# ChainBreak/denoising_diffusion_deep_fake

Hardware: NVIDIA B200
Metric: train_img_per_s (higher is better)
Workload: dtype bf16

## Files before the change

denoising_diffusion_deep_fake_b200/csrc/api.cu:

```cuda
#include <stdarg.h>
#include <string.h>
#include <stdlib.h>
#include "common.cuh"

namespace d3fk {

int64_t g_launch_count = 0;
char g_last_error[512] = "";
int* g_dev_error_flag = nullptr;
int g_use_pdl = 1;
static int g_inited_device = -1;

int set_error(int code, const char* fmt, ...) {
  va_list ap;
  va_start(ap, fmt);
  vsnprintf(g_last_error, sizeof(g_last_error), fmt, ap);
  va_end(ap);
  return code;
}

int check_launch(const char* what) {
  cudaError_t e = cudaPeekAtLastError();
  if (e != cudaSuccess) {
    cudaGetLastError();
// ... 27 lines not shown
int launch_chansum(const d3fk_chansum_params*, cudaStream_t);
int launch_upcat(const d3fk_upcat_params*, cudaStream_t);
int launch_frames_to_tensor(const d3fk_frames_params*, cudaStream_t);
int launch_tensor_to_frames(const d3fk_frames_params*, cudaStream_t);
int launch_affine_qsample(const d3fk_affine_qsample_params*, cudaStream_t);
int launch_qsample(const d3fk_qsample_params*, cudaStream_t);
int launch_posterior(const d3fk_posterior_params*, cudaStream_t);
int launch_inc(const d3fk_misc_params*, cudaStream_t);
int launch_adam(const d3fk_adam_params*, cudaStream_t);
int launch_set_scalars(const d3fk_scalars_params*, cudaStream_t);
int launch_pack_all(const d3fk_misc_params*, cudaStream_t);
int launch_loss(const d3fk_loss_params*, cudaStream_t);
int loss_init();
int tc_init();

static int require_init() {
  if (g_inited_device < 0) return set_error(D3FK_ERR_ARCH, "d3fk_init() has not succeeded on an sm_100 device");
  return D3FK_OK;
}

static int conv_dispatch(const d3fk_conv_params* p, cudaStream_t s) {
  if (p->dtype == D3FK_F32) {
    if (p->mode == 2) return set_error(D3FK_ERR_UNSUPPORTED, "conv mode 2 (windowed rows) is a bf16-engine path");
    return launch_conv_ffma(p, s);
  }
  if (p->dtype == D3FK_BF16) return launch_conv_tc(p, s);
  return set_error(D3FK_ERR_ARG, "conv: bad dtype %d", p->dtype);
}
static int wgrad_dispatch(const d3fk_wgrad_params* p, cudaStream_t s) {
  if (p->dtype == D3FK_F32) {
    if (p->mode == 2) return set_error(D3FK_ERR_UNSUPPORTED, "wgrad mode 2 (space-to-depth stem) is a bf16-engine path");
    return launch_wgrad_ffma(p, s);
  }
  if (p->dtype == D3FK_BF16) return launch_wgrad_tc(p, s);
  return set_error(D3FK_ERR_ARG, "wgrad: bad dtype %d", p->dtype);
}

static int wgrad_group_dispatch(const d3fk_wgrad_group_params* p, cudaStream_t s) {
  if (p->base.dtype == D3FK_BF16) return launch_wgrad_group_tc(p, s);
  if (p->count < 1 || p->count > D3FK_WGRAD_GROUP_MAX) return set_error(D3FK_ERR_ARG, "wgrad group: count %d", p->count);
  for (int i = 0; i < p->count; ++i) {
    d3fk_wgrad_params one = p->base;
    one.src0 = p->src0[i]; one.dy = p->dy[i]; one.dw = p->dw[i];
    int rc = wgrad_dispatch(&one, s);
    if (rc) return rc;
  }
// ... 297 lines not shown
```

denoising_diffusion_deep_fake_b200/csrc/conv_tc.cu:

```cuda
#include "tc_common.cuh"

namespace d3fk {

template <int BN, int PATH, int FUSE> struct ConvCfg {
  static constexpr int STAGES = BN >= 128 ? ((PATH == 2 && FUSE == 3) ? 6 : 3) : 4;
  static constexpr int B_STAGE_BYTES = BN * 128;
  static constexpr int SMEM = 1024 + STAGES * (A_STAGE_BYTES + B_STAGE_BYTES) + 256 + 10 * BN * 4;
  static constexpr int ACC_COLS = BN < 32 ? 32 : BN;
  static constexpr int TMEM_COLS = 2 * ACC_COLS;
};

struct TileSched {
  int MT, NT, KS, kb_per_split, nkb, total, a_ca;
  int bw, bh, bn, wt, ht;
  int off_w, off_h;
  int a_pitch;
};

__device__ __forceinline__ void decode_tile(const TileSched& ts, int t, int& mt, int& nt, int& ks) {
  if (ts.KS > 1) {
    ks = t % ts.KS;
    const int r = t / ts.KS;
    mt = r % ts.MT;
    nt = r / ts.MT;
  } else {
    ks = 0;
    mt = t % ts.MT;
    nt = t / ts.MT;
  }
}

struct FuseBN {
  const float* gamma; const float* beta;
  float* mean; float* invstd; float* running_mean; float* running_var; long long* nbt;
  float* scale; float* shift;
  bf16* act; const bf16* res;
  unsigned* barrier;
  long long count;
  int ldact, ldr, relu;
  float eps, momentum;
};

template <int BN, int PATH, int FUSE>
__global__ void __launch_bounds__(TC_THREADS, 2) conv_tc_kernel(Gather g, FastDiv dWo, FastDiv dHo, const __grid_constant__ CUtensorMap tmA,
                                                             const __grid_constant__ CUtensorMap tmB, EpiTC e, TileSched ts,
                                                             FuseBN fb, int* errflag) {
  using Cfg = ConvCfg<BN, PATH, FUSE>;
  constexpr int STAGES = Cfg::STAGES;
  constexpr int CW = BN >= 32 ? 32 : 16;
  extern __shared__ uint8_t smem_raw[];
  const uint32_t base = (smem_u32(smem_raw) + 1023u) & ~1023u;
  const uint32_t a_base = base;
  const uint32_t b_base = base + STAGES * A_STAGE_BYTES;
  const uint32_t bar_base = b_base + STAGES * Cfg::B_STAGE_BYTES;
  uint8_t* gen_bar = smem_raw + (base - smem_u32(smem_raw)) + STAGES * (A_STAGE_BYTES + Cfg::B_STAGE_BYTES);
  volatile uint32_t* tmem_ptr_slot = reinterpret_cast<volatile uint32_t*>(gen_bar + 8 * (2 * STAGES + 4));
  float* s_stat = reinterpret_cast<float*>(gen_bar + 256);
  float* s_aff = s_stat + 8 * BN;
  constexpr bool affine = FUSE == 3;
  auto full_bar = [&](int s) { return bar_base + 8u * s; };
  auto empty_bar = [&](int s) { return bar_base + 8u * (STAGES + s); };
  auto acc_full_bar = [&](int b) { return bar_base + 8u * (2 * STAGES + b); };
  auto acc_empty_bar = [&](int b) { return bar_base + 8u * (2 * STAGES + 2 + b); };
  const uint32_t recv_bar = bar_base + 8u * (2 * STAGES + 5);

  const int tid = threadIdx.x, warp = warp_index_uniform(), lane = tid & 31;
// ... 21 lines not shown
      mbar_init(empty_bar(s), 1);
    }
    for (int b = 0; b < 2; ++b) {
      mbar_init(acc_full_bar(b), 1);
      mbar_init(acc_empty_bar(b), EPI_THREADS);
    }
    mbar_init(recv_bar, 1);
    fence_barrier_init();
  }
  if (is_epi) {
    for (int i = etid; i < 8 * BN; i += EPI_THREADS) s_stat[i] = 0.f;
  }
  if (warp == 5 && elect_one_sync()) {
    tma_prefetch_desc(&tmB);
    if (PATH == 2) tma_prefetch_desc(&tmA);
    int mt0, nt0, ks0;
    decode_tile(ts, blockIdx.x, mt0, nt0, ks0);
    const int kbp = ks0 * ts.kb_per_split;
    for (int i = 0; i < STAGES && kbp + i < ts.nkb; ++i) tma_prefetch_l2_2d(&tmB, (kbp + i) * TC_BK, nt0 * BN);
  }
  if (FUSE == 2 && is_epi && e.bw_x) {
    int mt0, nt0, ks0;
    decode_tile(ts, blockIdx.x, mt0, nt0, ks0);
    const long long mp = (long long)mt0 * TC_BM + q * 32 + lane;
    if (mp < g.M) {
      for (int b = half * 128; b < BN * 2; b += 256) {
        prefetch_l2(reinterpret_cast<const char*>(e.bw_x + mp * e.bw_ldx + nt0 * BN) + b);
        if (e.bw_relu) prefetch_l2(reinterpret_cast<const char*>(e.bw_act + mp * e.bw_ldact + nt0 * BN) + b);
      }
    }
  }
  if (warp == 4) tmem_alloc(smem_u32((const void*)tmem_ptr_slot), Cfg::TMEM_COLS);
  tc_fence_before();
  __syncthreads();
  tc_fence_after();
  const uint32_t tmem_d = *tmem_ptr_slot;
  if (tid == 0) { TL_STAMP(1) }

  auto flush_stats = [&](int nt) {
    asm volatile("bar.sync 1, 256;" ::: "memory");
    const int n0 = nt * BN;
    if (tid < BN && n0 + tid < e.Cout) {
      const float a = (s_stat[tid] + s_stat[2 * BN + tid]) + (s_stat[4 * BN + tid] + s_stat[6 * BN + tid]);
      const float b = (s_stat[BN + tid] + s_stat[3 * BN + tid]) + (s_stat[5 * BN + tid] + s_stat[7 * BN + tid]);
      if (a != 0.f || b != 0.f) {
        atomicAdd(&e.stats[n0 + tid], (double)a);
        atomicAdd(&e.stats[e.Cout + n0 + tid], (FUSE == 2 && e.bw_x) ? bw_second_sum((double)a, (double)b, e, n0 + tid) : (double)b);
      }
// ... 46 lines not shown
        for (int i = 0; i < 8; ++i) y[i] += __bfloat162float(rb16[i]);
      }
      if (fb.relu) {
#pragma unroll
        for (int i = 0; i < 8; ++i) y[i] = fmaxf(y[i], 0.f);
      }
      uint4 o;
      __nv_bfloat162* o2 = reinterpret_cast<__nv_bfloat162*>(&o);
#pragma unroll
      for (int i = 0; i < 4; ++i) o2[i] = __floats2bfloat162_rn(y[2 * i], y[2 * i + 1]);
      *reinterpret_cast<uint4*>(fb.act + m * fb.ldact + cbase + q * 8) = o;
    }
  };

  if (warp == 5) {
    pdl_enter();
    if (tid == 160) { TL_STAMP(2) }
    if (elect_one_sync()) {
      uint32_t kbg = 0;
      const int sgn = g.mode ? -1 : 1;
      for (int t = blockIdx.x; t < ts.total; t += gridDim.x) {
        int mt, nt, ks;
        decode_tile(ts, t, mt, nt, ks);
        const int kb0 = ks * ts.kb_per_split;
        const int kb1 = min(ts.nkb, kb0 + ts.kb_per_split);
        int w0 = 0, h0 = 0, i0 = 0, tap = 0, c = 0, khi = 0, kwi = 0;
        if (PATH == 2) {
          const int tw = mt % ts.wt;
          const int r2 = mt / ts.wt;
          w0 = tw * ts.bw + ts.off_w;
          h0 = (r2 % ts.ht) * ts.bh + ts.off_h;
          i0 = (r2 / ts.ht) * ts.bn;
          const int k = kb0 * TC_BK;
          tap = k / g.ctot;
          c = k - tap * g.ctot;
          khi = tap / g.kw;
          kwi = tap - khi * g.kw;
        }
        for (int kb = kb0; kb < kb1; ++kb, ++kbg) {
          const int s = kbg % STAGES;
          if (kbg >= STAGES) mbar_wait(empty_bar(s), ((kbg / STAGES) - 1) & 1, errflag);
          mbar_arrive_expect_tx(full_bar(s), Cfg::B_STAGE_BYTES + (PATH == 2 ? A_STAGE_BYTES : 0));
          tma_load_2d(b_base + s * Cfg::B_STAGE_BYTES, &tmB, kb * TC_BK, nt * BN, full_bar(s));
          if (PATH == 2) {
            tma_load_4d(a_base + s * A_STAGE_BYTES, &tmA, c, w0 + sgn * kwi, h0 + sgn * khi, i0, full_bar(s));
            c += TC_BK;
            if (c >= g.ctot) {
              c = 0;
              if (++kwi == g.kw) { kwi = 0; ++khi; }
            }
          }
        }
      }
    }
    __syncwarp();
    if (clus) cluster_sync_relaxed();
  } else if (warp == 4) {
    pdl_enter();
    if (elect_one_sync()) {
      constexpr uint32_t idesc = make_idesc(TC_BM, BN, 0, 0);
      uint32_t kbg = 0, tile_iter = 0;
      for (int t = blockIdx.x; t < ts.total; t += gridDim.x, ++tile_iter) {
        int mt, nt, ks;
        decode_tile(ts, t, mt, nt, ks);
        const int kb0 = ks * ts.kb_per_split;
        const int kb1 = min(ts.nkb, kb0 + ts.kb_per_split);
        const uint32_t abuf = tile_iter & 1;
        if (tile_iter >= 2) {
          mbar_wait(acc_empty_bar(abuf), ((tile_iter >> 1) - 1) & 1, errflag);
          tc_fence_after();
        }
        const uint32_t d_addr = tmem_d + abuf * Cfg::ACC_COLS;
        for (int kb = kb0; kb < kb1; ++kb, ++kbg) {
          const int s = kbg % STAGES;
          mbar_wait(full_bar(s), (kbg / STAGES) & 1, errflag);
          if (kbg == 0) { TL_STAMP(3) }
          tc_fence_after();
          const uint32_t a_addr = a_base + s * A_STAGE_BYTES;
          const uint32_t b_addr = b_base + s * Cfg::B_STAGE_BYTES;
#pragma unroll
          for (int kk = 0; kk < TC_BK / 16; ++kk) {
            uint64_t ad = make_smem_desc(a_addr + kk * 32, 16, 1024);
            uint64_t bd = make_smem_desc(b_addr + kk * 32, 16, 1024);
            umma_f16(d_addr, ad, bd, idesc, (kb > kb0 || kk > 0) ? 1u : 0u);
          }
          umma_commit(empty_bar(s));
        }
        umma_commit(acc_full_bar(abuf));
        TL_STAMP(4)
      }
    }
    __syncwarp();
    if (clus) cluster_sync_relaxed();
  } else {
    const int j = tid & 7;
    const int rb = tid >> 3;
    const uint32_t sw = (uint32_t)((j ^ (rb & 7)) << 4);
    const int sgn = g.mode ? -1 : 1;
    const uint32_t smask = g.mode ? (uint32_t)(g.stride - 1) : 0u;
    const int sshift = g.mode ? g.sshift : 0;
    const int row = q * 32 + lane;
#pragma unroll 1
    for (int pass = 0; pass < 2; ++pass) {
      int pass_v = pass;
      asm volatile("" : "+r"(pass_v));
      const bool live = pass_v != 0;
      if (live) {
        pdl_enter();
        if (tid == 0) { TL_STAMP(2) }
      }
      uint32_t kbg = 0;
      uint32_t tile_iter = 0;
      int cur_nt = -1, cur_aff_nt = -1;
      for (int t = blockIdx.x; t < ts.total; t += gridDim.x, ++tile_iter) {
        int mt, nt, ks;
        decode_tile(ts, t, mt, nt, ks);
        const int m0 = mt * TC_BM, n0 = nt * BN;
        const int kb0 = ks * ts.kb_per_split;
        const int kb1 = min(ts.nkb, kb0 + ts.kb_per_split);

        if (PATH != 2 && warp < 4 && live) {
          int rh[8], rw[8];
          int rn[8];
          const bf16* rp[8];
#pragma unroll
          for (int i = 0; i < 8; ++i) {
            const int m = m0 + rb + 16 * i;
            int n = 0, h0 = -(1 << 28), w0 = 0;
            if (m < g.M) {
              const uint32_t qq = fdiv((uint32_t)m, dWo);
              const int wo = m - (int)qq * g.Wo;
              n = (int)fdiv(qq, dHo);
              const int ho = (int)qq - n * g.Ho;
              if (g.mode == 0) { h0 = ho * g.stride - g.pad; w0 = wo * g.stride - g.pad; }
              else { h0 = ho + g.pad; w0 = wo + g.pad; }
            }
            rh[i] = h0; rw[i] = w0;
            if (PATH == 0) rp[i] = (const bf16*)g.src0 + ((long long)(n * g.Hi + h0) * g.Wi + w0) * g.ld0;
            else rn[i] = n;
          }
          int k = kb0 * TC_BK + j * 8;
          int tap = k / g.ctot;
// ... 31 lines not shown
                if (ts.a_ca) cp_async_16_ca(a_dst + i * (16 * 128), src, ok ? 16u : 0u);
                else cp_async_16(a_dst + i * (16 * 128), src, ok ? 16u : 0u);
              }
            }
            cp_async_mbar_arrive(full_bar(s));
            mbar_arrive(full_bar(s));
            k += TC_BK;
            c += TC_BK;
            while (c >= g.ctot) {
              c -= g.ctot;
              if (++kwi == g.kw) { kwi = 0; ++khi; }
            }
          }
        }

        const uint32_t abuf = tile_iter & 1;
        if (live) {
          mbar_wait(acc_full_bar(abuf), (tile_iter >> 1) & 1, errflag);
          if (tid == 0) { TL_STAMP(5) }
          tc_fence_after();
        }
        const int m = m0 + row;
        const bool row_ok = live && m < g.M;
        if (!clus) {
          if (affine && (cur_aff_nt != nt || !live)) {
            stage_affine(nt, live);
            cur_aff_nt = live ? nt : -1;
          }
          if (live && do_stats && cur_nt != nt) {
            if (cur_nt >= 0) flush_stats(cur_nt);
            cur_nt = nt;
          }
          int on = 0, oh = 0, ow = 0;
          if (e.out_nchw && row_ok) {
            const uint32_t qq = fdiv((uint32_t)m, dWo);
            ow = m - (int)qq * e.Wo;
            on = (int)fdiv(qq, dHo);
            oh = (int)qq - on * e.Ho;
          }
#pragma unroll 1
          for (int cc = half * CW; cc < BN; cc += 2 * CW) {
            uint32_t raw[CW];
            const uint32_t taddr = tmem_d + ((uint32_t)(q * 32) << 16) + abuf * Cfg::ACC_COLS + (uint32_t)cc;
            const bool tstats = do_stats && !(FUSE == 2 && e.bw_x);
            if (tstats) tmem_col_stats<CW>(taddr, live ? g.M - (m0 + q * 32) : 0, s_stat + q * 2 * BN + cc, s_stat + q * 2 * BN + BN + cc, lane);
            if (CW == 32) tmem_ld32(taddr, raw); else tmem_ld16(taddr, raw);
            tmem_ld_wait();
            float f[CW];
#pragma unroll
            for (int i = 0; i < CW; ++i) f[i] = __uint_as_float(raw[i]);
            epilogue_chunk<CW, FUSE == 2>(f, e, (long long)m, row_ok, n0 + cc, on, oh, ow, do_stats && !tstats, s_stat + q * 2 * BN + cc,
                                          s_stat + q * 2 * BN + BN + cc, lane, affine ? s_aff + cc : nullptr, BN);
            if (tid == 0 && cc == 0) { TL_STAMP(8) }
          }
          if (tid == 0) { TL_STAMP(9) }
          if (FUSE == 1 && live) {
            flush_stats(nt);
            cur_nt = -1;
            fuse_finalize(nt, mt == 0);
#pragma unroll 1
            for (int cc = half * CW; cc < BN; cc += 2 * CW) {
              uint32_t raw[CW];
              const uint32_t taddr = tmem_d + ((uint32_t)(q * 32) << 16) + abuf * Cfg::ACC_COLS + (uint32_t)cc;
              if (CW == 32) tmem_ld32(taddr, raw); else tmem_ld16(taddr, raw);
              tmem_ld_wait();
              float f[CW];
#pragma unroll
              for (int i = 0; i < CW; ++i) f[i] = __uint_as_float(raw[i]);
              fuse_apply(f, CW, (long long)m, row_ok, nt, cc);
            }
          }
          if (live) {
            tc_fence_before();
            mbar_arrive(acc_empty_bar(abuf));
          }
        } else {
          const int KS = ts.KS, SL = BN / KS, sl4 = SL >> 2;
          const uint32_t rank = cluster_ctarank();
          const uint32_t recv = a_base;
          if (live) {
            if (etid == 0) mbar_arrive_expect_tx(recv_bar, (uint32_t)(TC_BM * BN * 4));
            tc_fence_before();
            cluster_sync_relaxed();
            tc_fence_after();
            if (tid == 0) { TL_STAMP(11) }
          }
#pragma unroll 1
          for (int cc = half * CW; cc < BN; cc += 2 * CW) {
            uint32_t raw[CW];
            const uint32_t taddr = tmem_d + ((uint32_t)(q * 32) << 16) + (uint32_t)cc;
            if (CW == 32) tmem_ld32(taddr, raw); else tmem_ld16(taddr, raw);
            tmem_ld_wait();
#pragma unroll
            for (int q4 = 0; q4 < CW / 4; ++q4) {
              const int col = cc + 4 * q4;
              const int owner = col / SL, within = col - owner * SL;
              const uint32_t la = recv + (uint32_t)((((int)rank * sl4 + (within >> 2)) * 128 + row) * 16);
              const uint32_t ra = mapa_shared(la, (uint32_t)owner);
              if (live) st_async_f4(ra, raw[4 * q4], raw[4 * q4 + 1], raw[4 * q4 + 2], raw[4 * q4 + 3], mapa_shared(recv_bar, (uint32_t)owner));
            }
          }
          if (live) {
            if (tid == 0) { TL_STAMP(12) }
            mbar_wait(recv_bar, 0, errflag);
            if (tid == 0) { TL_STAMP(13) }
          }
          if (affine) stage_affine(nt, live);
          const int cslice = (int)rank * SL;
#pragma unroll 1
          for (int ch = half * 16; ch < SL; ch += 32) {
            float f[16];
#pragma unroll
            for (int c4 = 0; c4 < 4; ++c4) {
              float4 a = make_float4(0.f, 0.f, 0.f, 0.f);
              for (int r = 0; r < KS; ++r) {
                const float4 v = ld_shared_f4(recv + (uint32_t)(((r * sl4 + (ch >> 2) + c4) * 128 + row) * 16));
                a.x += v.x; a.y += v.y; a.z += v.z; a.w += v.w;
              }
              f[4 * c4] = a.x; f[4 * c4 + 1] = a.y; f[4 * c4 + 2] = a.z; f[4 * c4 + 3] = a.w;
            }
            const int ct = cslice + ch;
            const bool tstats = do_stats && !(FUSE == 2 && e.bw_x);
            if (tstats) {
              const uint32_t taddr = tmem_d + ((uint32_t)(q * 32) << 16) + (uint32_t)ct;
              if (live) tmem_st16(taddr, f);
              __syncwarp();
              tmem_col_stats<16>(taddr, live ? g.M - (m0 + q * 32) : 0, s_stat + q * 2 * BN + ct, s_stat + q * 2 * BN + BN + ct, lane);
            }
            epilogue_chunk<16, FUSE == 2>(f, e, (long long)m, row_ok, nt * BN + ct, 0, 0, 0, do_stats && !tstats, s_stat + q * 2 * BN + ct,
                                          s_stat + q * 2 * BN + BN + ct, lane, affine ? s_aff + ct : nullptr, BN);
          }
          if (tid == 0) { TL_STAMP(14) }
          if (live && do_stats) flush_stats(nt);
          if (tid == 0) { TL_STAMP(15) }
          if (FUSE == 1 && live) {
            fuse_finalize(nt, mt == 0 && rank == 0);
#pragma unroll 1
            for (int ch = half * 16; ch < SL; ch += 32) {
              float f[16];
#pragma unroll
              for (int c4 = 0; c4 < 4; ++c4) {
                float4 a = make_float4(0.f, 0.f, 0.f, 0.f);
                for (int r = 0; r < KS; ++r) {
                  const float4 v = ld_shared_f4(recv + (uint32_t)(((r * sl4 + (ch >> 2) + c4) * 128 + row) * 16));
                  a.x += v.x; a.y += v.y; a.z += v.z; a.w += v.w;
                }
                f[4 * c4] = a.x; f[4 * c4 + 1] = a.y; f[4 * c4 + 2] = a.z; f[4 * c4 + 3] = a.w;
              }
              fuse_apply(f, 16, (long long)m, row_ok, nt, cslice + ch);
            }
          }
        }
// ... 5 lines not shown
  }

  if (tid == 0) { TL_STAMP(6) }
  tc_fence_before();
  __syncthreads();
  if (warp == 4) tmem_dealloc(tmem_d, Cfg::TMEM_COLS);
  if (tid == 128) { TL_STAMP(7) }
}

int g_num_sms = 148;
int g_verbose = 0;
int g_max_cluster = 8;
static int g_tile_loop = 1;
static int g_a_ca = 0;
static int g_occ_cap = 0;
static int g_use_tma_a = 1;
static int g_split_tiles = 74;
static int g_split_cta_cap = 100;

struct FuseReq { const d3fk_bn_params* bn; unsigned* barrier; bool taken; };
static thread_local FuseReq* t_fuse = nullptr;
static int g_fuse_bn = 1;

template <int BN, int PATH>
static int launch_conv_tc_bn(const Gather& g, const d3fk_conv_params* p, cudaStream_t s, const TileSched& box) {
  EpiTC e{(bf16*)p->out, p->out_nchw, p->scale, p->shift, (const bf16*)p->res, p->stats, p->ldo, p->ldr, p->relu, p->Cout, p->Ho, p->Wo,
           (const bf16*)p->bw_x, (const bf16*)p->bw_act, p->bw_mean, p->bw_invstd, p->bw_ldx, p->bw_ldact, p->bw_relu};
  TileSched ts = box;
  ts.MT = cdiv(g.M, TC_BM);
  ts.NT = cdiv(p->Cout, BN);
  ts.nkb = cdiv(g.K, TC_BK);
  ts.KS = 1;
  const int tiles = ts.MT * ts.NT;
  ts.a_ca = g_a_ca && p->kh > 1;
  if (BN == 128 && !p->out_nchw && p->Cout % BN == 0 && tiles <= g_split_tiles && ts.nkb >= 8 && g_max_cluster > 1) {
    int ks = 1;
    while (ks * 2 <= g_max_cluster && ks * 2 <= 8 && tiles * ks * 2 <= g_split_cta_cap * g_num_sms / 100 && ts.nkb / (ks * 2) >= 4) ks *= 2;
    while (ks > 1 && tiles * ks > cluster_capacity(ks, 2)) ks >>= 1;
    ts.KS = ks;
  }
  ts.kb_per_split = cdiv(ts.nkb, ts.KS);
  if (ts.KS > 1 && (ts.KS - 1) * ts.kb_per_split >= ts.nkb) {
    ts.KS = 1;
    ts.kb_per_split = ts.nkb;
  }
  ts.total = tiles * ts.KS;
  const bool eval_affine = !p->bw_x && (p->scale || p->shift);
  const int smem_bytes = eval_affine ? ConvCfg<BN, PATH, 3>::SMEM : ConvCfg<BN, PATH, 0>::SMEM;
  int occ = (227 * 1024) / (smem_bytes + 1024);
  if (occ * ConvCfg<BN, PATH, 0>::TMEM_COLS > 512) occ = 512 / ConvCfg<BN, PATH, 0>::TMEM_COLS;
  if (g_occ_cap > 0 && occ > g_occ_cap) occ = g_occ_cap;
  int grid = ts.total < g_num_sms * occ ? ts.total : g_num_sms * occ;
  if (!g_tile_loop || ts.KS > 1) grid = ts.total;

  alignas(64) CUtensorMap tmA, tmB;
  memset(&tmA, 0, sizeof(tmA));
  {
    uint64_t dims[2] = {(uint64_t)g.K, (uint64_t)p->Cout};
    uint64_t strides[1] = {(uint64_t)g.K * 2};
    uint32_t bx[2] = {TC_BK, (uint32_t)BN};
// ... 3 lines not shown
  if (PATH == 2) {
    uint64_t dims[4] = {(uint64_t)g.c0, (uint64_t)g.Wi, (uint64_t)g.Hi, (uint64_t)g.B};
    const uint64_t pitch = (uint64_t)(ts.a_pitch ? ts.a_pitch : g.Wi);
    uint64_t strides[3] = {(uint64_t)g.ld0 * 2, pitch * g.ld0 * 2, (uint64_t)g.Hi * pitch * g.ld0 * 2};
    uint32_t bx[4] = {TC_BK, (uint32_t)ts.bw, (uint32_t)ts.bh, (uint32_t)ts.bn};
    int rc = get_tensor_map(&tmA, p->src0, 4, dims, strides, bx, 128);
    if (rc) return rc;
  }
  FuseBN fb;
  memset(&fb, 0, sizeof(fb));
  bool fuse = false;
  if (BN == 128 && t_fuse && g_fuse_bn && p->stats && !p->scale && !p->shift && !p->res && !p->relu && !p->out_nchw && p->mode == 0 &&
      p->Cout % BN == 0 && ts.total <= cluster_capacity_safe(ts.KS)) {
    const d3fk_bn_params* b = t_fuse->bn;
    fb.gamma = b->gamma; fb.beta = b->beta; fb.mean = b->mean; fb.invstd = b->invstd; fb.scale = b->scale; fb.shift = b->shift;
    fb.running_mean = b->running_mean; fb.running_var = b->running_var; fb.nbt = (long long*)b->num_batches_tracked;
    fb.act = (bf16*)b->y; fb.res = (const bf16*)b->res; fb.barrier = t_fuse->barrier; fb.count = b->count;
    fb.ldact = b->ldy; fb.ldr = b->ldr; fb.relu = b->relu; fb.eps = b->eps; fb.momentum = b->momentum;
    fuse = true;
    grid = ts.total;
    t_fuse->taken = true;
  }
  const int epi = p->bw_x ? 2 : fuse ? 1 : (p->scale || p->shift) ? 3 : 0;
  if (g_verbose) fprintf(stderr, "[d3fk] conv<%d,%d> mode=%d M=%d K=%d Cout=%d tiles=%d KS=%d kbps=%d grid=%d fuse=%d epi=%d\n", BN, PATH, g.mode, g.M, g.K, p->Cout, tiles, ts.KS, ts.kb_per_split, grid, (int)fuse, epi);
  cudaError_t le;
  if (p->bw_x)
    le = launch_k(conv_tc_kernel<BN, PATH, 2>, dim3(grid), dim3(TC_THREADS), ConvCfg<BN, PATH, 2>::SMEM, s, dim3(ts.KS, 1, 1), g,
                  make_fastdiv((uint32_t)g.Wo), make_fastdiv((uint32_t)g.Ho), tmA, tmB, e, ts, fb, g_dev_error_flag);
  else if (BN == 128 && fuse)
    le = launch_k(conv_tc_kernel<BN, PATH, (BN == 128 ? 1 : 0)>, dim3(grid), dim3(TC_THREADS), ConvCfg<BN, PATH, 1>::SMEM, s, dim3(ts.KS, 1, 1), g,
                  make_fastdiv((uint32_t)g.Wo), make_fastdiv((uint32_t)g.Ho), tmA, tmB, e, ts, fb, g_dev_error_flag);
  else if (p->scale || p->shift)
    le = launch_k(conv_tc_kernel<BN, PATH, 3>, dim3(grid), dim3(TC_THREADS), ConvCfg<BN, PATH, 3>::SMEM, s, dim3(ts.KS, 1, 1), g,
                  make_fastdiv((uint32_t)g.Wo), make_fastdiv((uint32_t)g.Ho), tmA, tmB, e, ts, fb, g_dev_error_flag);
  else
    le = launch_k(conv_tc_kernel<BN, PATH, 0>, dim3(grid), dim3(TC_THREADS), ConvCfg<BN, PATH, 0>::SMEM, s, dim3(ts.KS, 1, 1), g,
                  make_fastdiv((uint32_t)g.Wo), make_fastdiv((uint32_t)g.Ho), tmA, tmB, e, ts, fb, g_dev_error_flag);
  if (le != cudaSuccess) return set_error(D3FK_ERR_CUDA, "conv_tc launch: %s", cudaGetErrorString(le));
  count_launch();
  return check_launch("conv_tc");
}

template <int PATH>
static int launch_conv_tc_path(const Gather& g, const d3fk_conv_params* p, cudaStream_t s, const TileSched& box) {
  const int C = p->Cout;
  if (C <= 16) return launch_conv_tc_bn<16, PATH>(g, p, s, box);
  D3FK_CHECK_ARG(p->out_nchw == nullptr, "out_nchw only for Cout <= 16");
  if (C % 128 == 0) return launch_conv_tc_bn<128, PATH>(g, p, s, box);
  if (C % 64 == 0) return launch_conv_tc_bn<64, PATH>(g, p, s, box);
  if (C % 32 == 0) return launch_conv_tc_bn<32, PATH>(g, p, s, box);
  return set_error(D3FK_ERR_UNSUPPORTED, "conv_tc: Cout=%d (need <=16 or a multiple of 32)", C);
}

static bool tma_box(const Gather& g, const d3fk_conv_params* p, TileSched& ts) {
  if (!g_use_tma_a) return false;
  if (p->c1 != 0 || p->up0 != 0 || p->stride != 1 || g.ctot % TC_BK != 0) return false;
  if (p->Ho != p->Hi || p->Wo != p->Wi || 2 * p->pad != p->kh - 1 || p->kh != p->kw) return false;
  if (((uintptr_t)p->src0 & 15) || (g.ld0 % 8)) return false;
  const int W = p->Wi, H = p->Hi;
// ... 12 lines not shown
  return true;
}

static int launch_conv_windowed(const d3fk_conv_params* p, cudaStream_t s) {
  D3FK_CHECK_ARG(p->c0 == 64 && p->c1 == 0 && p->ld0 == 16 && p->kh == 4 && p->kw == 1 && p->stride == 1 && p->up0 == 0,
                 "conv mode 2: c0 = 64, ld0 = 16, 4 x 1 taps, stride 1");
  D3FK_CHECK_ARG(p->Ho == p->Hi && p->Wo == p->Wi && p->Cout == 64 && !p->out_nchw && !p->bw_x, "conv mode 2: Ho = Hi, Wo = Wi, Cout = 64");
  d3fk_conv_params q = *p;
  q.mode = 0;
  Gather g;
  int rc = make_gather(g, q.src0, nullptr, q.c0, 0, q.ld0, 0, 0, q.B, q.Hi, q.Wi, q.Ho, q.Wo, q.kh, q.kw, 1, q.pad, 0);
  if (rc) return rc;
  TileSched box;
  memset(&box, 0, sizeof(box));
  q.pad = 0; q.kh = q.kw = 1;
  if (!tma_box(g, &q, box)) return set_error(D3FK_ERR_UNSUPPORTED, "conv mode 2: the 128-pixel tile is not a (w, h, n) box for %d x %d", p->Ho, p->Wo);
  q.pad = p->pad; q.kh = p->kh; q.kw = p->kw;
  box.off_w = 0;
  box.off_h = -p->pad;
  box.a_pitch = p->Wi + 3;
  return launch_conv_tc_bn<64, 2>(g, &q, s, box);
}

int try_launch_conv_slab(const Gather& g, const d3fk_conv_params* p, cudaStream_t s);
int try_launch_head_conv(const d3fk_conv_params* p, cudaStream_t s);
int launch_conv_tc(const d3fk_conv_params* p, cudaStream_t s) {
  Gather g;
  int rc = make_gather(g, p->src0, p->src1, p->c0, p->c1, p->ld0, p->ld1, p->up0, p->B, p->Hi, p->Wi, p->Ho, p->Wo, p->kh,
                       p->kw, p->stride, p->pad, p->mode);
  if (rc) return rc;
  D3FK_CHECK_ARG(p->out || p->out_nchw, "no output");
  D3FK_CHECK_ARG(p->out_nchw || (p->ldo % 8 == 0), "ldo must be a multiple of 8");
  D3FK_CHECK_ARG(!p->scale || p->shift, "scale requires shift");
  D3FK_CHECK_ARG(((uintptr_t)p->w & 15) == 0, "weights must be 16-byte aligned");
  if (p->mode == 2) return launch_conv_windowed(p, s);
  const int head = try_launch_head_conv(p, s);
  if (head) return head < 0 ? head : D3FK_OK;
  const int slab = try_launch_conv_slab(g, p, s);
  if (slab) return slab < 0 ? slab : D3FK_OK;
  TileSched box;
  memset(&box, 0, sizeof(box));
  if (tma_box(g, p, box)) return launch_conv_tc_path<2>(g, p, s, box);
  const bool linear = p->c1 == 0 && p->up0 == 0 && (p->mode == 0 || p->stride == 1);
  return linear ? launch_conv_tc_path<0>(g, p, s, box) : launch_conv_tc_path<1>(g, p, s, box);
}

int launch_bn_apply(const d3fk_bn_params* p, cudaStream_t s);
int launch_conv_bn_tc(const d3fk_convbn_params* p, cudaStream_t s) {
  FuseReq req{&p->bn, (unsigned*)p->barrier, false};
// ... 42 lines not shown
  D3FK_SET_SMEM((conv_tc_kernel<32, 1, 2>), (ConvCfg<32, 1, 2>::SMEM))
  D3FK_SET_SMEM((conv_tc_kernel<32, 2, 2>), (ConvCfg<32, 2, 2>::SMEM))
  D3FK_SET_SMEM((conv_tc_kernel<64, 0, 2>), (ConvCfg<64, 0, 2>::SMEM))
  D3FK_SET_SMEM((conv_tc_kernel<64, 1, 2>), (ConvCfg<64, 1, 2>::SMEM))
  D3FK_SET_SMEM((conv_tc_kernel<64, 2, 2>), (ConvCfg<64, 2, 2>::SMEM))
  D3FK_SET_SMEM((conv_tc_kernel<128, 0, 2>), (ConvCfg<128, 0, 2>::SMEM))
  D3FK_SET_SMEM((conv_tc_kernel<128, 1, 2>), (ConvCfg<128, 1, 2>::SMEM))
  D3FK_SET_SMEM((conv_tc_kernel<128, 2, 2>), (ConvCfg<128, 2, 2>::SMEM))
  D3FK_SET_SMEM((conv_tc_kernel<128, 0, 1>), (ConvCfg<128, 0, 1>::SMEM))
  D3FK_SET_SMEM((conv_tc_kernel<128, 1, 1>), (ConvCfg<128, 1, 1>::SMEM))
  D3FK_SET_SMEM((conv_tc_kernel<128, 2, 1>), (ConvCfg<128, 2, 1>::SMEM))
  D3FK_SET_SMEM((conv_tc_kernel<16, 0, 3>), (ConvCfg<16, 0, 3>::SMEM))
  D3FK_SET_SMEM((conv_tc_kernel<16, 1, 3>), (ConvCfg<16, 1, 3>::SMEM))
  D3FK_SET_SMEM((conv_tc_kernel<16, 2, 3>), (ConvCfg<16, 2, 3>::SMEM))
  D3FK_SET_SMEM((conv_tc_kernel<32, 0, 3>), (ConvCfg<32, 0, 3>::SMEM))
  D3FK_SET_SMEM((conv_tc_kernel<32, 1, 3>), (ConvCfg<32, 1, 3>::SMEM))
  D3FK_SET_SMEM((conv_tc_kernel<32, 2, 3>), (ConvCfg<32, 2, 3>::SMEM))
  D3FK_SET_SMEM((conv_tc_kernel<64, 0, 3>), (ConvCfg<64, 0, 3>::SMEM))
  D3FK_SET_SMEM((conv_tc_kernel<64, 1, 3>), (ConvCfg<64, 1, 3>::SMEM))
  D3FK_SET_SMEM((conv_tc_kernel<64, 2, 3>), (ConvCfg<64, 2, 3>::SMEM))
  D3FK_SET_SMEM((conv_tc_kernel<128, 0, 3>), (ConvCfg<128, 0, 3>::SMEM))
  D3FK_SET_SMEM((conv_tc_kernel<128, 1, 3>), (ConvCfg<128, 1, 3>::SMEM))
  D3FK_SET_SMEM((conv_tc_kernel<128, 2, 3>), (ConvCfg<128, 2, 3>::SMEM))
  if (e != cudaSuccess) return set_error(D3FK_ERR_CUDA, "cudaFuncSetAttribute: %s", cudaGetErrorString(e));
  int rc = slab_init();
  if (rc) return rc;
  return wgrad_init();
}

}
```

denoising_diffusion_deep_fake_b200/plan.py:

```python
import os

import torch

from . import _lib
from ._lib import make_op, op_params

_f = int(os.environ.get("D3FK_FUSE_BNBW", "1100000"))
FUSE_BN_BWD_MAX_ELEMS = (1 << 62) if _f == 1 else _f
GROUP_WGRAD = os.environ.get("D3FK_WGRAD_GROUP", "0") == "1"
GROUP_WGRAD_SIZE = int(os.environ.get("D3FK_WGRAD_GROUP_SIZE", "0"))

UPCAT_ALL = os.environ.get("D3FK_UPCAT_ALL", "1") == "1"

BRANCH_LANE = int(os.environ.get("D3FK_BRANCH_LANE", "1"))

BN_EPS = 1e-5
BN_MOMENTUM = 0.1
SPLITK_WS_BYTES = 64 << 20
CIN_PAD = 8
DY_PAD = 16


class ConvSpec:
    def __init__(self, name, cin, cout, k, stride, pad, bn=None, bias=False):
# ... 399 lines not shown

    def _flush_wgrad_group(self, ops, pending):
        if not pending:
            return
        if len(pending) == 1:
            c, src, dy = pending[0]
            ops.append(self._wgrad_op(c, src, None, 0, dy))
        else:
            c, src, dy = pending[0]
            for c2, s2, d2 in pending[1:]:
                assert (c2.k, c2.stride, c2.pad, c2.cin, c2.cout, s2.H, s2.W, s2.C, s2.ld, d2.H, d2.W, d2.C, d2.ld) == \
                       (c.k, c.stride, c.pad, c.cin, c.cout, src.H, src.W, src.C, src.ld, dy.H, dy.W, dy.C, dy.ld)
            base = dict(dtype=self.dtype, c0=src.C, ld0=src.ld, up0=0, B=self.B, Hi=src.H, Wi=src.W, Ho=dy.H, Wo=dy.W,
                        kh=c.k, kw=c.k, stride=c.stride, pad=c.pad, ldy=dy.ld, Cout=dy.C, cin_real=c.cin, cout_real=c.cout)
            ops.append(make_op(_lib.OP_WGRAD_GROUP, base=base, count=len(pending),
                               src0=[s2.ptr for _, s2, _ in pending], dy=[d2.ptr for _, _, d2 in pending],
                               dw=[self._gptr(c2.name + ".weight") for c2, _, _ in pending]))
        pending.clear()

    def _dgrad_op(self, c, dy, out, res=None, row0=0, rows=None, lane=0):
        cout_pad = dy.C
        rows = out.C if rows is None else rows
        wbytes = 4 if self.dtype == _lib.F32 else 2
        f = dict(dtype=self.dtype, mode=1, src0=dy.ptr, c0=dy.C, ld0=dy.ld, B=self.B, Hi=dy.H, Wi=dy.W,
                 Ho=out.H, Wo=out.W, kh=c.k, kw=c.k, stride=c.stride, pad=c.pad,
                 w=self.w_dgrad[c.name].data_ptr() + row0 * c.k * c.k * cout_pad * wbytes, Cout=rows,
                 out=out.ptr, ldo=out.ld)
        if self.ws is not None:
            f.update(ws=self.ws.data_ptr(), ws_bytes=SPLITK_WS_BYTES)
        if res is not None:
            f.update(res=res.ptr, ldr=res.ld)
        return make_op(_lib.OP_CONV, lane=lane, **f)

    def _bn_bwd(self, ops, c, g_act, want_dres=False, lane=0):
        sv = self.saved[c.name]
        raw, act = sv["raw"], sv["act"]
        d_raw = T(self, raw.B, raw.H, raw.W, raw.C)
        self.keep.append(d_raw.t)
        bn = dict(sv["bn"])
        bn.update(dy=g_act.ptr, lddy=g_act.ld, act=act.ptr, ldact=act.ld, dx=d_raw.ptr, lddx=d_raw.ld,
                  dgamma=self._gptr(c.bn + ".weight"), dbeta=self._gptr(c.bn + ".bias"))
        g_masked = None
        if want_dres:
            g_masked = T(self, raw.B, raw.H, raw.W, raw.C)
            self.keep.append(g_masked.t)
            bn.update(dres=g_masked.ptr, lddres=g_masked.ld)
        bn["mask_from_x"] = 1 if (sv["res"] is None and sv["relu"]) else 0
        bn.pop("res", None)
        bn.pop("ldr", None)
        fuse = self.dtype == _lib.BF16 and raw.B * raw.H * raw.W * raw.C <= FUSE_BN_BWD_MAX_ELEMS
        prod = self._grad_producer.get(id(g_act)) if fuse else None
        if prod is not None:
            pp = op_params(prod)
            pp.stats = bn["bstats"]
            pp.bw_x, pp.bw_ldx = raw.ptr, raw.ld
# ... 136 lines not shown
```

Before: 74010.

## Add parity-class decomposition for stride-2 3x3 dgrad convolutions

Adds conv mode 4, which computes the data gradient of a stride-2, pad-1 3x3 convolution as four output-parity classes. Each class only iterates over the taps that contribute to it, so the zero-inserted taps of the transposed conv are not multiplied, and each class is fed by TMA box loads of the dense dy tensor. The epilogue remaps class-local rows to interleaved output pixels, and classes with an empty K range write zeros. The planner selects this path for eligible bf16 dgrad ops. The cost is extra index math, uneven work across the four classes, and a new split-K heuristic.

New measurement: 74510, median of 6. No clear change (+0.7%).

```diff
diff --git a/denoising_diffusion_deep_fake_b200/csrc/api.cu b/denoising_diffusion_deep_fake_b200/csrc/api.cu
--- a/denoising_diffusion_deep_fake_b200/csrc/api.cu
+++ b/denoising_diffusion_deep_fake_b200/csrc/api.cu
@@ -73,6 +73,7 @@
 static int conv_dispatch(const d3fk_conv_params* p, cudaStream_t s) {
   if (p->dtype == D3FK_F32) {
     if (p->mode == 2) return set_error(D3FK_ERR_UNSUPPORTED, "conv mode 2 (windowed rows) is a bf16-engine path");
+    if (p->mode == 4) return set_error(D3FK_ERR_UNSUPPORTED, "conv mode 4 (parity classes) is a bf16-engine path");
     return launch_conv_ffma(p, s);
   }
   if (p->dtype == D3FK_BF16) return launch_conv_tc(p, s);
diff --git a/denoising_diffusion_deep_fake_b200/csrc/conv_tc.cu b/denoising_diffusion_deep_fake_b200/csrc/conv_tc.cu
--- a/denoising_diffusion_deep_fake_b200/csrc/conv_tc.cu
+++ b/denoising_diffusion_deep_fake_b200/csrc/conv_tc.cu
@@ -15,7 +15,46 @@
   int bw, bh, bn, wt, ht;
   int off_w, off_h;
   int a_pitch;
+  int cls_mt;
 };
+
+__device__ __forceinline__ int par_class(const TileSched& ts, int mt) { return 3 - mt / ts.cls_mt; }
+
+__device__ __forceinline__ int par_count(int pq, int cb, int x) {
+  const int p = pq >> 1, q = pq & 1;
+  int n = 0;
+  for (int a = 0; a <= p; ++a)
+    for (int b = 0; b <= q; ++b) {
+      const int tap = (p ? 2 * a : 1) * 3 + (q ? 2 * b : 1);
+      n += min(max(x - tap * cb, 0), cb);
+    }
+  return n;
+}
+
+template <bool PAR>
+__device__ __forceinline__ void tile_krange(const TileSched& ts, const Gather& g, int mt, int ks, int& kb0, int& kb1) {
+  const int lo = ks * ts.kb_per_split;
+  const int hi = min(ts.nkb, lo + ts.kb_per_split);
+  if (PAR) {
+    const int pq = par_class(ts, mt), cb = g.ctot / TC_BK;
+    kb0 = par_count(pq, cb, lo);
+    kb1 = par_count(pq, cb, hi);
+  } else {
+    kb0 = lo;
+    kb1 = hi;
+  }
+}
+
+__device__ __forceinline__ long long out_pixel(const TileSched& ts, const EpiTC& e, FastDiv dWo, FastDiv dHo, int Hc, int Wc,
+                                               int mt, int ml) {
+  if (!ts.cls_mt) return ml;
+  const int pq = par_class(ts, mt);
+  const uint32_t r = fdiv((uint32_t)ml, dWo);
+  const int j = ml - (int)r * Wc;
+  const int n = (int)fdiv(r, dHo);
+  const int i = (int)r - n * Hc;
+  return ((long long)n * e.Ho + 2 * i + (pq >> 1)) * e.Wo + 2 * j + (pq & 1);
+}
 
 __device__ __forceinline__ void decode_tile(const TileSched& ts, int t, int& mt, int& nt, int& ks) {
   if (ts.KS > 1) {
@@ -41,7 +80,7 @@
   float eps, momentum;
 };
 
-template <int BN, int PATH, int FUSE>
+template <int BN, int PATH, int FUSE, bool PAR = false>
 __global__ void __launch_bounds__(TC_THREADS, 2) conv_tc_kernel(Gather g, FastDiv dWo, FastDiv dHo, const __grid_constant__ CUtensorMap tmA,
                                                              const __grid_constant__ CUtensorMap tmB, EpiTC e, TileSched ts,
                                                              FuseBN fb, int* errflag) {
@@ -109,8 +148,9 @@
   if (FUSE == 2 && is_epi && e.bw_x) {
     int mt0, nt0, ks0;
     decode_tile(ts, blockIdx.x, mt0, nt0, ks0);
-    const long long mp = (long long)mt0 * TC_BM + q * 32 + lane;
-    if (mp < g.M) {
+    const int ml = (PAR ? (mt0 % ts.cls_mt) : mt0) * TC_BM + q * 32 + lane;
+    if (ml < g.M) {
+      const long long mp = PAR ? out_pixel(ts, e, dWo, dHo, g.Ho, g.Wo, mt0, ml) : ml;
       for (int b = half * 128; b < BN * 2; b += 256) {
         prefetch_l2(reinterpret_cast<const char*>(e.bw_x + mp * e.bw_ldx + nt0 * BN) + b);
         if (e.bw_relu) prefetch_l2(reinterpret_cast<const char*>(e.bw_act + mp * e.bw_ldact + nt0 * BN) + b);
@@ -203,12 +243,13 @@
       for (int t = blockIdx.x; t < ts.total; t += gridDim.x) {
         int mt, nt, ks;
         decode_tile(ts, t, mt, nt, ks);
-        const int kb0 = ks * ts.kb_per_split;
-        const int kb1 = min(ts.nkb, kb0 + ts.kb_per_split);
+        int kb0, kb1;
+        tile_krange<PAR>(ts, g, mt, ks, kb0, kb1);
         int w0 = 0, h0 = 0, i0 = 0, tap = 0, c = 0, khi = 0, kwi = 0;
         if (PATH == 2) {
-          const int tw = mt % ts.wt;
-          const int r2 = mt / ts.wt;
+          const int mtl = PAR ? mt % ts.cls_mt : mt;
+          const int tw = mtl % ts.wt;
+          const int r2 = mtl / ts.wt;
           w0 = tw * ts.bw + ts.off_w;
           h0 = (r2 % ts.ht) * ts.bh + ts.off_h;
           i0 = (r2 / ts.ht) * ts.bn;
@@ -222,6 +263,16 @@
           const int s = kbg % STAGES;
           if (kbg >= STAGES) mbar_wait(empty_bar(s), ((kbg / STAGES) - 1) & 1, errflag);
           mbar_arrive_expect_tx(full_bar(s), Cfg::B_STAGE_BYTES + (PATH == 2 ? A_STAGE_BYTES : 0));
+          if (PAR) {
+            const int pq = par_class(ts, mt), cb = g.ctot / TC_BK;
+            const int tap_i = kb / cb, ntw = 1 + (pq & 1);
+            const int a = tap_i / ntw, b = tap_i - a * ntw;
+            const int kh = (pq >> 1) ? 2 * a : 1, kw = (pq & 1) ? 2 * b : 1;
+            c = (kb - tap_i * cb) * TC_BK;
+            tma_load_2d(b_base + s * Cfg::B_STAGE_BYTES, &tmB, (kh * 3 + kw) * g.ctot + c, nt * BN, full_bar(s));
+            tma_load_4d(a_base + s * A_STAGE_BYTES, &tmA, c, w0 + ((pq & 1) && kw == 0), h0 + ((pq >> 1) && kh == 0), i0, full_bar(s));
+            continue;
+          }
           tma_load_2d(b_base + s * Cfg::B_STAGE_BYTES, &tmB, kb * TC_BK, nt * BN, full_bar(s));
           if (PATH == 2) {
             tma_load_4d(a_base + s * A_STAGE_BYTES, &tmA, c, w0 + sgn * kwi, h0 + sgn * khi, i0, full_bar(s));
@@ -244,8 +295,8 @@
       for (int t = blockIdx.x; t < ts.total; t += gridDim.x, ++tile_iter) {
         int mt, nt, ks;
         decode_tile(ts, t, mt, nt, ks);
-        const int kb0 = ks * ts.kb_per_split;
-        const int kb1 = min(ts.nkb, kb0 + ts.kb_per_split);
+        int kb0, kb1;
+        tile_krange<PAR>(ts, g, mt, ks, kb0, kb1);
         const uint32_t abuf = tile_iter & 1;
         if (tile_iter >= 2) {
           mbar_wait(acc_empty_bar(abuf), ((tile_iter >> 1) - 1) & 1, errflag);
@@ -267,7 +318,8 @@
           }
           umma_commit(empty_bar(s));
         }
-        umma_commit(acc_full_bar(abuf));
+        if (PAR && kb0 == kb1) mbar_arrive(acc_full_bar(abuf));
+        else umma_commit(acc_full_bar(abuf));
         TL_STAMP(4)
       }
     }
@@ -296,9 +348,9 @@
       for (int t = blockIdx.x; t < ts.total; t += gridDim.x, ++tile_iter) {
         int mt, nt, ks;
         decode_tile(ts, t, mt, nt, ks);
-        const int m0 = mt * TC_BM, n0 = nt * BN;
-        const int kb0 = ks * ts.kb_per_split;
-        const int kb1 = min(ts.nkb, kb0 + ts.kb_per_split);
+        const int m0 = (PAR ? mt % ts.cls_mt : mt) * TC_BM, n0 = nt * BN;
+        int kb0, kb1;
+        tile_krange<PAR>(ts, g, mt, ks, kb0, kb1);
 
         if (PATH != 2 && warp < 4 && live) {
           int rh[8], rw[8];
@@ -376,6 +428,7 @@
         }
         const int m = m0 + row;
         const bool row_ok = live && m < g.M;
+        const long long mo = PAR && row_ok ? out_pixel(ts, e, dWo, dHo, g.Ho, g.Wo, mt, m) : m;
         if (!clus) {
           if (affine && (cur_aff_nt != nt || !live)) {
             stage_affine(nt, live);
@@ -403,7 +456,7 @@
             float f[CW];
 #pragma unroll
             for (int i = 0; i < CW; ++i) f[i] = __uint_as_float(raw[i]);
-            epilogue_chunk<CW, FUSE == 2>(f, e, (long long)m, row_ok, n0 + cc, on, oh, ow, do_stats && !tstats, s_stat + q * 2 * BN + cc,
+            epilogue_chunk<CW, FUSE == 2>(f, e, mo, row_ok, n0 + cc, on, oh, ow, do_stats && !tstats, s_stat + q * 2 * BN + cc,
                                           s_stat + q * 2 * BN + BN + cc, lane, affine ? s_aff + cc : nullptr, BN);
             if (tid == 0 && cc == 0) { TL_STAMP(8) }
           }
@@ -445,6 +498,10 @@
             const uint32_t taddr = tmem_d + ((uint32_t)(q * 32) << 16) + (uint32_t)cc;
             if (CW == 32) tmem_ld32(taddr, raw); else tmem_ld16(taddr, raw);
             tmem_ld_wait();
+            if (PAR && kb0 == kb1) {
+#pragma unroll
+              for (int i = 0; i < CW; ++i) raw[i] = 0u;
+            }
 #pragma unroll
             for (int q4 = 0; q4 < CW / 4; ++q4) {
               const int col = cc + 4 * q4;
@@ -481,7 +538,7 @@
               __syncwarp();
               tmem_col_stats<16>(taddr, live ? g.M - (m0 + q * 32) : 0, s_stat + q * 2 * BN + ct, s_stat + q * 2 * BN + BN + ct, lane);
             }
-            epilogue_chunk<16, FUSE == 2>(f, e, (long long)m, row_ok, nt * BN + ct, 0, 0, 0, do_stats && !tstats, s_stat + q * 2 * BN + ct,
+            epilogue_chunk<16, FUSE == 2>(f, e, mo, row_ok, nt * BN + ct, 0, 0, 0, do_stats && !tstats, s_stat + q * 2 * BN + ct,
                                           s_stat + q * 2 * BN + BN + ct, lane, affine ? s_aff + ct : nullptr, BN);
           }
           if (tid == 0) { TL_STAMP(14) }
@@ -533,20 +590,21 @@
 static thread_local FuseReq* t_fuse = nullptr;
 static int g_fuse_bn = 1;
 
-template <int BN, int PATH>
+template <int BN, int PATH, bool PAR = false>
 static int launch_conv_tc_bn(const Gather& g, const d3fk_conv_params* p, cudaStream_t s, const TileSched& box) {
   EpiTC e{(bf16*)p->out, p->out_nchw, p->scale, p->shift, (const bf16*)p->res, p->stats, p->ldo, p->ldr, p->relu, p->Cout, p->Ho, p->Wo,
            (const bf16*)p->bw_x, (const bf16*)p->bw_act, p->bw_mean, p->bw_invstd, p->bw_ldx, p->bw_ldact, p->bw_relu};
   TileSched ts = box;
-  ts.MT = cdiv(g.M, TC_BM);
+  ts.MT = ts.cls_mt ? 4 * ts.cls_mt : cdiv(g.M, TC_BM);
   ts.NT = cdiv(p->Cout, BN);
   ts.nkb = cdiv(g.K, TC_BK);
   ts.KS = 1;
   const int tiles = ts.MT * ts.NT;
+  const int tiles1 = ts.cls_mt ? cdiv(4 * g.M, TC_BM) * ts.NT : tiles;
   ts.a_ca = g_a_ca && p->kh > 1;
-  if (BN == 128 && !p->out_nchw && p->Cout % BN == 0 && tiles <= g_split_tiles && ts.nkb >= 8 && g_max_cluster > 1) {
+  if (BN == 128 && !p->out_nchw && p->Cout % BN == 0 && tiles1 <= g_split_tiles && ts.nkb >= 8 && g_max_cluster > 1) {
     int ks = 1;
-    while (ks * 2 <= g_max_cluster && ks * 2 <= 8 && tiles * ks * 2 <= g_split_cta_cap * g_num_sms / 100 && ts.nkb / (ks * 2) >= 4) ks *= 2;
+    while (ks * 2 <= g_max_cluster && ks * 2 <= 8 && tiles1 * ks * 2 <= g_split_cta_cap * g_num_sms / 100 && ts.nkb / (ks * 2) >= 4) ks *= 2;
     while (ks > 1 && tiles * ks > cluster_capacity(ks, 2)) ks >>= 1;
     ts.KS = ks;
   }
@@ -596,19 +654,19 @@
     t_fuse->taken = true;
   }
   const int epi = p->bw_x ? 2 : fuse ? 1 : (p->scale || p->shift) ? 3 : 0;
-  if (g_verbose) fprintf(stderr, "[d3fk] conv<%d,%d> mode=%d M=%d K=%d Cout=%d tiles=%d KS=%d kbps=%d grid=%d fuse=%d epi=%d\n", BN, PATH, g.mode, g.M, g.K, p->Cout, tiles, ts.KS, ts.kb_per_split, grid, (int)fuse, epi);
+  if (g_verbose) fprintf(stderr, "[d3fk] conv<%d,%d> mode=%d M=%d K=%d Cout=%d tiles=%d KS=%d kbps=%d grid=%d fuse=%d epi=%d geom=%d\n", BN, PATH, g.mode, g.M, g.K, p->Cout, tiles, ts.KS, ts.kb_per_split, grid, (int)fuse, epi, ts.cls_mt ? 4 : ts.a_pitch ? 2 : g.mode);
   cudaError_t le;
   if (p->bw_x)
-    le = launch_k(conv_tc_kernel<BN, PATH, 2>, dim3(grid), dim3(TC_THREADS), ConvCfg<BN, PATH, 2>::SMEM, s, dim3(ts.KS, 1, 1), g,
+    le = launch_k(conv_tc_kernel<BN, PATH, 2, PAR>, dim3(grid), dim3(TC_THREADS), ConvCfg<BN, PATH, 2>::SMEM, s, dim3(ts.KS, 1, 1), g,
                   make_fastdiv((uint32_t)g.Wo), make_fastdiv((uint32_t)g.Ho), tmA, tmB, e, ts, fb, g_dev_error_flag);
   else if (BN == 128 && fuse)
-    le = launch_k(conv_tc_kernel<BN, PATH, (BN == 128 ? 1 : 0)>, dim3(grid), dim3(TC_THREADS), ConvCfg<BN, PATH, 1>::SMEM, s, dim3(ts.KS, 1, 1), g,
+    le = launch_k(conv_tc_kernel<BN, PATH, (BN == 128 ? 1 : 0), PAR>, dim3(grid), dim3(TC_THREADS), ConvCfg<BN, PATH, 1>::SMEM, s, dim3(ts.KS, 1, 1), g,
                   make_fastdiv((uint32_t)g.Wo), make_fastdiv((uint32_t)g.Ho), tmA, tmB, e, ts, fb, g_dev_error_flag);
   else if (p->scale || p->shift)
-    le = launch_k(conv_tc_kernel<BN, PATH, 3>, dim3(grid), dim3(TC_THREADS), ConvCfg<BN, PATH, 3>::SMEM, s, dim3(ts.KS, 1, 1), g,
+    le = launch_k(conv_tc_kernel<BN, PATH, 3, PAR>, dim3(grid), dim3(TC_THREADS), ConvCfg<BN, PATH, 3>::SMEM, s, dim3(ts.KS, 1, 1), g,
                   make_fastdiv((uint32_t)g.Wo), make_fastdiv((uint32_t)g.Ho), tmA, tmB, e, ts, fb, g_dev_error_flag);
   else
-    le = launch_k(conv_tc_kernel<BN, PATH, 0>, dim3(grid), dim3(TC_THREADS), ConvCfg<BN, PATH, 0>::SMEM, s, dim3(ts.KS, 1, 1), g,
+    le = launch_k(conv_tc_kernel<BN, PATH, 0, PAR>, dim3(grid), dim3(TC_THREADS), ConvCfg<BN, PATH, 0>::SMEM, s, dim3(ts.KS, 1, 1), g,
                   make_fastdiv((uint32_t)g.Wo), make_fastdiv((uint32_t)g.Ho), tmA, tmB, e, ts, fb, g_dev_error_flag);
   if (le != cudaSuccess) return set_error(D3FK_ERR_CUDA, "conv_tc launch: %s", cudaGetErrorString(le));
   count_launch();
@@ -667,9 +725,34 @@
   return launch_conv_tc_bn<64, 2>(g, &q, s, box);
 }
 
+static int launch_conv_parity(const d3fk_conv_params* p, cudaStream_t s) {
+  D3FK_CHECK_ARG(p->kh == 3 && p->kw == 3 && p->stride == 2 && p->pad == 1 && p->c1 == 0 && p->up0 == 0 && !p->out_nchw,
+                 "conv mode 4: 3 x 3 taps, stride 2, pad 1, one source, NHWC output");
+  D3FK_CHECK_ARG(p->Ho == 2 * p->Hi && p->Wo == 2 * p->Wi, "conv mode 4: Ho = 2 Hi, Wo = 2 Wi");
+  D3FK_CHECK_ARG(p->Cout % 128 == 0 && !p->scale && !p->shift, "conv mode 4: Cout a multiple of 128 (128-wide tiles), no scale / shift");
+  d3fk_conv_params q = *p;
+  q.mode = 1;
+  Gather g;
+  int rc = make_gather(g, q.src0, nullptr, q.c0, 0, q.ld0, 0, 0, q.B, q.Hi, q.Wi, q.Hi, q.Wi, 3, 3, 1, 1, 1);
+  if (rc) return rc;
+  TileSched box;
+  memset(&box, 0, sizeof(box));
+  q.stride = 1; q.Ho = q.Hi; q.Wo = q.Wi;
+  if (!tma_box(g, &q, box))
+    return set_error(D3FK_ERR_UNSUPPORTED, "conv mode 4: needs c0 %% 64 == 0, a 16-byte aligned src0 and a (w, h, n) box on %d x %d", p->Hi, p->Wi);
+  box.off_w = box.off_h = 0;
+  box.cls_mt = cdiv(g.M, TC_BM);
+  return launch_conv_tc_bn<128, 2, true>(g, p, s, box);
+}
+
 int try_launch_conv_slab(const Gather& g, const d3fk_conv_params* p, cudaStream_t s);
 int try_launch_head_conv(const d3fk_conv_params* p, cudaStream_t s);
 int launch_conv_tc(const d3fk_conv_params* p, cudaStream_t s) {
+  D3FK_CHECK_ARG((p->mode >= 0 && p->mode <= 2) || p->mode == 4, "conv: mode must be 0, 1, 2 or 4");
+  if (p->mode == 4) {
+    D3FK_CHECK_ARG(p->out && p->ldo % 8 == 0 && ((uintptr_t)p->w & 15) == 0, "conv mode 4: out with ldo a multiple of 8, 16-byte aligned weights");
+    return launch_conv_parity(p, s);
+  }
   Gather g;
   int rc = make_gather(g, p->src0, p->src1, p->c0, p->c1, p->ld0, p->ld1, p->up0, p->B, p->Hi, p->Wi, p->Ho, p->Wo, p->kh,
                        p->kw, p->stride, p->pad, p->mode);
@@ -758,6 +841,8 @@
   D3FK_SET_SMEM((conv_tc_kernel<128, 0, 3>), (ConvCfg<128, 0, 3>::SMEM))
   D3FK_SET_SMEM((conv_tc_kernel<128, 1, 3>), (ConvCfg<128, 1, 3>::SMEM))
   D3FK_SET_SMEM((conv_tc_kernel<128, 2, 3>), (ConvCfg<128, 2, 3>::SMEM))
+  D3FK_SET_SMEM((conv_tc_kernel<128, 2, 0, true>), (ConvCfg<128, 2, 0>::SMEM))
+  D3FK_SET_SMEM((conv_tc_kernel<128, 2, 2, true>), (ConvCfg<128, 2, 2>::SMEM))
   if (e != cudaSuccess) return set_error(D3FK_ERR_CUDA, "cudaFuncSetAttribute: %s", cudaGetErrorString(e));
   int rc = slab_init();
   if (rc) return rc;
diff --git a/denoising_diffusion_deep_fake_b200/plan.py b/denoising_diffusion_deep_fake_b200/plan.py
--- a/denoising_diffusion_deep_fake_b200/plan.py
+++ b/denoising_diffusion_deep_fake_b200/plan.py
@@ -445,7 +445,8 @@
         cout_pad = dy.C
         rows = out.C if rows is None else rows
         wbytes = 4 if self.dtype == _lib.F32 else 2
-        f = dict(dtype=self.dtype, mode=1, src0=dy.ptr, c0=dy.C, ld0=dy.ld, B=self.B, Hi=dy.H, Wi=dy.W,
+        mode = 4 if self._parity_dgrad(c, dy, out, rows) else 1
+        f = dict(dtype=self.dtype, mode=mode, src0=dy.ptr, c0=dy.C, ld0=dy.ld, B=self.B, Hi=dy.H, Wi=dy.W,
                  Ho=out.H, Wo=out.W, kh=c.k, kw=c.k, stride=c.stride, pad=c.pad,
                  w=self.w_dgrad[c.name].data_ptr() + row0 * c.k * c.k * cout_pad * wbytes, Cout=rows,
                  out=out.ptr, ldo=out.ld)
@@ -454,6 +455,11 @@
         if res is not None:
             f.update(res=res.ptr, ldr=res.ld)
         return make_op(_lib.OP_CONV, lane=lane, **f)
+
+    def _parity_dgrad(self, c, dy, out, rows):
+        return (self.dtype == _lib.BF16 and c.k == 3 and c.stride == 2 and c.pad == 1 and rows % 128 == 0
+                and dy.C % 64 == 0 and dy.ld % 8 == 0 and dy.ptr % 16 == 0 and out.H == 2 * dy.H and out.W == 2 * dy.W
+                and self._stem_box_ok(dy.H, dy.W))
 
     def _bn_bwd(self, ops, c, g_act, want_dres=False, lane=0):
         sv = self.saved[c.name]
```
